# arpitbansal297/Cold-Diffusion-Models

Hardware: AMD Instinct MI355X
Metric: unet_train_imgs_per_sec (higher is better)
Workload: dtype f32 storage/accumulate; dense-conv GEMM operands bf16x3; 1 GPU; CelebA-128 denoising cold diffusion (BASELINE config 3): Unet(dim=64,(1,2,4,8),ch=3) @128x128, T=200, optimizer step = 2 micro-batches x 32 img (one fused forward / backward pass over all of them: same draws, same gradient sum) + Adam + EMA/10; per_gpu_batch=32, gradient_accumulate_every=2, parallelism=single

## Files before the change

cold-diffusion-models_amd/csrc/k_pack.hip:

```cpp
#include "cdf_common.h"
#include "colddiff.h"

__global__ void pack_weight_kernel(const float* src, float* dst, int T, int R, int C, int ldc, long long s_t,
                                   long long s_r, long long s_c) {
    const long long n = (long long)T * R * ldc;
    for (long long i = (long long)blockIdx.x * blockDim.x + threadIdx.x; i < n; i += (long long)gridDim.x * blockDim.x) {
        const int c = (int)(i % ldc);
        const long long tr = i / ldc;
        const int r = (int)(tr % R), t = (int)(tr / R);
        dst[i] = c < C ? src[c * s_c + r * s_r + t * s_t] : 0.f;
    }
}

__global__ void pack_weight_bf16_kernel(const float* src, unsigned short* dst_hi, unsigned short* dst_lo, int T, int R, int C,
                                        int ldc, long long s_t, long long s_r, long long s_c) {
    const long long n = (long long)T * R * ldc;
    for (long long i = (long long)blockIdx.x * blockDim.x + threadIdx.x; i < n; i += (long long)gridDim.x * blockDim.x) {
        const int c = (int)(i % ldc);
        const long long tr = i / ldc;
        const int r = (int)(tr % R), t = (int)(tr / R);
        const float v = c < C ? src[c * s_c + r * s_r + t * s_t] : 0.f;
        const unsigned h = cdf_f2bf(v);
        dst_hi[i] = (unsigned short)h;
        if (dst_lo) dst_lo[i] = (unsigned short)cdf_f2bf(v - cdf_bf2f(h));
    }
}

__global__ void split_bf16_kernel(const float* x, int ldx, unsigned short* hi, unsigned short* lo, int ldo, long long rows, int C4) {
    const long long n = rows * C4;
    for (long long i = (long long)blockIdx.x * blockDim.x + threadIdx.x; i < n; i += (long long)gridDim.x * blockDim.x) {
        const int c = (int)(i % C4) * 4;
        const long long r = i / C4;
        const float4 v = *(const float4*)(x + r * ldx + c);
        uint2 h, l;
        cdf_split4(v.x, v.y, v.z, v.w, h, l);
        *(uint2*)(hi + r * ldo + c) = h;
        if (lo) *(uint2*)(lo + r * ldo + c) = l;
    }
}

__global__ void widen_bf16_kernel(const unsigned short* x, int ldx, float* y, int ldy, long long rows, int C4) {
    const long long n = rows * C4;
    for (long long i = (long long)blockIdx.x * blockDim.x + threadIdx.x; i < n; i += (long long)gridDim.x * blockDim.x) {
        const int c = (int)(i % C4) * 4;
        const long long r = i / C4;
        *(float4*)(y + r * ldy + c) = cdf_quad_cvt(*(const uint2*)(x + r * ldx + c));
    }
}

struct CdfPackEntry {
    const float* src;
    void* dst0;
    void* dst1;
    long long s_t, s_r, s_c;
    int T, R, C, ldc, kind, first_block;
};

__global__ void __launch_bounds__(256) pack_many_kernel(const CdfPackEntry* tab, int nentries) {
    int lo = 0, hi = nentries - 1;
    const int b = blockIdx.x;
    while (lo < hi) {
        const int mid = (lo + hi + 1) >> 1;
        if (tab[mid].first_block <= b) lo = mid; else hi = mid - 1;
    }
    const CdfPackEntry e = tab[lo];
    if (e.s_t == 1 && e.T > 1 && e.T <= 16) {
        const long long n2 = (long long)e.R * e.ldc;
        const long long j0 = (long long)(b - e.first_block) * 1024 + threadIdx.x;
        const long long plane = (long long)e.R * e.ldc;
#pragma unroll
        for (int k = 0; k < 4; ++k) {
            const long long j = j0 + 256 * k;
            if (j >= n2) break;
            const int c = (int)(j % e.ldc), r = (int)(j / e.ldc);
            const bool ok = c < e.C;
            const float* sp = e.src + (ok ? c * e.s_c + r * e.s_r : 0);
            float v[16];
#pragma unroll
            for (int t = 0; t < 16; ++t) v[t] = sp[t < e.T ? t : 0];
#pragma unroll
            for (int t = 0; t < 16; ++t) {
                if (t >= e.T) break;
                const float x = ok ? v[t] : 0.f;
                const long long i = t * plane + j;
                if (e.kind == 0) {
                    ((float*)e.dst0)[i] = x;
                } else {
                    const unsigned h = cdf_f2bf(x);
                    ((unsigned short*)e.dst0)[i] = (unsigned short)h;
                    if (e.dst1) ((unsigned short*)e.dst1)[i] = (unsigned short)cdf_f2bf(x - cdf_bf2f(h));
                }
            }
        }
        return;
    }
    const long long n = (long long)e.T * e.R * e.ldc;
    const long long i0 = (long long)(b - e.first_block) * 1024 + threadIdx.x;
#pragma unroll
    for (int k = 0; k < 4; ++k) {
        const long long i = i0 + 256 * k;
        if (i >= n) break;
        const int c = (int)(i % e.ldc);
        const long long tr = i / e.ldc;
        const int r = (int)(tr % e.R), t = (int)(tr / e.R);
        const float v = c < e.C ? e.src[c * e.s_c + r * e.s_r + t * e.s_t] : 0.f;
        if (e.kind == 0) {
            ((float*)e.dst0)[i] = v;
        } else {
            const unsigned h = cdf_f2bf(v);
            ((unsigned short*)e.dst0)[i] = (unsigned short)h;
            if (e.dst1) ((unsigned short*)e.dst1)[i] = (unsigned short)cdf_f2bf(v - cdf_bf2f(h));
        }
    }
}

extern "C" int cdf_pack_entry_bytes(void) { return (int)sizeof(CdfPackEntry); }
extern "C" int cdf_pack_blocks(int T, int R, int ldc, long long s_t) {
    const long long n = (s_t == 1 && T > 1 && T <= 16) ? (long long)R * ldc : (long long)T * R * ldc;
    return (int)((n + 1023) / 1024);
}

extern "C" int cdf_pack_many(const void* table, int nentries, int nblocks, void* stream) {
    CDF_REQUIRE(table && nentries > 0 && nblocks > 0, "cdf_pack_many: bad args");
    CDF_LAUNCH(pack_many_kernel, dim3(nblocks), dim3(256), 0, CDF_S, (const CdfPackEntry*)table, nentries);
    return cdf_check_launch("pack_many");
}

extern "C" int cdf_pack_weight(const float* src, float* dst, int T, int R, int C, int ldc, long long s_t,
                               long long s_r, long long s_c, void* stream) {
    CDF_REQUIRE(src && dst && T > 0 && R > 0 && C > 0 && ldc >= C && ldc % 4 == 0, "cdf_pack_weight: bad args");
    CDF_LAUNCH(pack_weight_kernel, dim3(cdf_ew_grid4k((long long)T * R * ldc)), dim3(256), 0, CDF_S, src, dst, T, R, C, ldc, s_t, s_r, s_c);
    return cdf_check_launch("pack_weight");
}

extern "C" int cdf_pack_weight_bf16(const float* src, void* dst_hi, void* dst_lo, int T, int R, int C, int ldc, long long s_t,
                                    long long s_r, long long s_c, void* stream) {
    CDF_REQUIRE(src && dst_hi && T > 0 && R > 0 && C > 0 && ldc >= C && ldc % 32 == 0, "cdf_pack_weight_bf16: bad args (ldc must be a multiple of 32)");
    long long g = ((long long)T * R * ldc + 255) / 256;
    if (g > 4096) g = 4096;
    CDF_LAUNCH(pack_weight_bf16_kernel, dim3((int)g), dim3(256), 0, CDF_S, src, (unsigned short*)dst_hi, (unsigned short*)dst_lo, T, R, C, ldc, s_t, s_r, s_c);
    return cdf_check_launch("pack_weight_bf16");
}

extern "C" int cdf_split_bf16(const float* x, int ldx, void* hi, void* lo, int ldo, long long rows, int C, void* stream) {
    CDF_REQUIRE(x && hi && rows > 0 && C > 0 && C % 4 == 0 && ldx % 4 == 0 && ldo % 8 == 0 && ldo >= C, "cdf_split_bf16: bad args (C %% 4, ldo %% 8)");
    long long g = (rows * (C / 4) + 255) / 256;
    if (g > 8192) g = 8192;
    CDF_LAUNCH(split_bf16_kernel, dim3((int)g), dim3(256), 0, CDF_S, x, ldx, (unsigned short*)hi, (unsigned short*)lo, ldo, rows, C / 4);
    return cdf_check_launch("split_bf16");
}

extern "C" int cdf_bf16_to_f32(const void* x, int ldx, float* y, int ldy, long long rows, int C, void* stream) {
    CDF_REQUIRE(x && y && rows > 0 && C > 0 && C % 4 == 0 && ldx % 4 == 0 && ldy % 4 == 0 && ldx >= C && ldy >= C && (((uintptr_t)x) & 7) == 0 &&
                (((uintptr_t)y) & 15) == 0, "cdf_bf16_to_f32: bad args (C %% 4, pitches %% 4, x 8-byte / y 16-byte aligned)");
    long long g = (rows * (C / 4) + 255) / 256;
    if (g > 8192) g = 8192;
    CDF_LAUNCH(widen_bf16_kernel, dim3((int)g), dim3(256), 0, CDF_S, (const unsigned short*)x, ldx, y, ldy, rows, C / 4);
    return cdf_check_launch("bf16_to_f32");
}
```

Before: 1334 img/s.

## Tile weight packing through shared memory for coalesced reads and vector writes

Replaces the per-element strided gather in the batched weight-pack kernel with a 3D tiled transpose staged in shared memory. The loop dimensions are sorted by source stride so global reads stay as contiguous as possible, and the output is written as float4 or packed uint4 bf16 hi/lo vectors. The aim is to cut uncoalesced memory traffic when converting weights into GEMM layouts each step. It adds shared-memory use, more index arithmetic and a different block-count formula that the host side must stay consistent with.

```diff
diff --git a/cold-diffusion-models_amd/csrc/k_pack.hip b/cold-diffusion-models_amd/csrc/k_pack.hip
--- a/cold-diffusion-models_amd/csrc/k_pack.hip
+++ b/cold-diffusion-models_amd/csrc/k_pack.hip
@@ -56,7 +56,17 @@
     int T, R, C, ldc, kind, first_block;
 };
 
+#define PACK_TC 32
+#define PACK_ROWS 288
+#define PACK_LP (PACK_TC + 1)
+static __host__ __device__ inline void pack_tile(int T, int& RE, int& TE) {
+    TE = T < 64 ? T : 64;
+    RE = PACK_ROWS / TE;
+    if (RE > 128) RE = 128;
+}
+
 __global__ void __launch_bounds__(256) pack_many_kernel(const CdfPackEntry* tab, int nentries) {
+    __shared__ float tile[PACK_ROWS * PACK_LP];
     int lo = 0, hi = nentries - 1;
     const int b = blockIdx.x;
     while (lo < hi) {
@@ -64,60 +74,124 @@
         if (tab[mid].first_block <= b) lo = mid; else hi = mid - 1;
     }
     const CdfPackEntry e = tab[lo];
-    if (e.s_t == 1 && e.T > 1 && e.T <= 16) {
-        const long long n2 = (long long)e.R * e.ldc;
-        const long long j0 = (long long)(b - e.first_block) * 1024 + threadIdx.x;
-        const long long plane = (long long)e.R * e.ldc;
-#pragma unroll
-        for (int k = 0; k < 4; ++k) {
-            const long long j = j0 + 256 * k;
-            if (j >= n2) break;
-            const int c = (int)(j % e.ldc), r = (int)(j / e.ldc);
-            const bool ok = c < e.C;
-            const float* sp = e.src + (ok ? c * e.s_c + r * e.s_r : 0);
-            float v[16];
-#pragma unroll
-            for (int t = 0; t < 16; ++t) v[t] = sp[t < e.T ? t : 0];
-#pragma unroll
-            for (int t = 0; t < 16; ++t) {
-                if (t >= e.T) break;
-                const float x = ok ? v[t] : 0.f;
-                const long long i = t * plane + j;
-                if (e.kind == 0) {
-                    ((float*)e.dst0)[i] = x;
-                } else {
-                    const unsigned h = cdf_f2bf(x);
-                    ((unsigned short*)e.dst0)[i] = (unsigned short)h;
-                    if (e.dst1) ((unsigned short*)e.dst1)[i] = (unsigned short)cdf_f2bf(x - cdf_bf2f(h));
+    int RE, TE;
+    pack_tile(e.T, RE, TE);
+    const int tiles_c = (e.ldc + PACK_TC - 1) / PACK_TC, tiles_r = (e.R + RE - 1) / RE;
+    int bid = b - e.first_block;
+    const int c0 = (bid % tiles_c) * PACK_TC;
+    bid /= tiles_c;
+    const int r0 = (bid % tiles_r) * RE, t0 = (bid / tiles_r) * TE;
+    const int tid = threadIdx.x;
+
+    {
+        int e0 = PACK_TC, e1 = RE, e2 = TE;
+        int s0 = (int)e.s_c, s1 = (int)e.s_r, s2 = (int)e.s_t;
+        int l0 = 1, l1 = PACK_LP, l2 = RE * PACK_LP;
+        int m0 = e.C - c0, m1 = e.R - r0, m2 = e.T - t0;
+        auto key = [](int s, int ext) { return ext == 1 ? 0x7fffffff : s; };
+        auto cswap = [&](int& ea, int& sa, int& la, int& ma, int& eb, int& sb, int& lb, int& mb) {
+            if (key(sb, eb) < key(sa, ea)) {
+                int t_;
+                t_ = ea; ea = eb; eb = t_;
+                t_ = sa; sa = sb; sb = t_;
+                t_ = la; la = lb; lb = t_;
+                t_ = ma; ma = mb; mb = t_;
+            }
+        };
+        cswap(e0, s0, l0, m0, e1, s1, l1, m1);
+        cswap(e1, s1, l1, m1, e2, s2, l2, m2);
+        cswap(e0, s0, l0, m0, e1, s1, l1, m1);
+        const int n = PACK_TC * RE * TE;
+        int a0 = tid % e0, a1 = (tid / e0) % e1, a2 = tid / (e0 * e1);
+        const int d0 = 256 % e0, d1 = (256 / e0) % e1, d2 = 256 / (e0 * e1);
+        const float* sp = e.C > c0 ? e.src + ((long long)c0 * e.s_c + (long long)r0 * e.s_r + (long long)t0 * e.s_t) : e.src;
+        const int D = d0 * s0 + d1 * s1 + d2 * s2, W0 = s1 - e0 * s0, W1 = s2 - e1 * s1;
+        const int DL = d0 * l0 + d1 * l1 + d2 * l2, WL0 = l1 - e0 * l0, WL1 = l2 - e1 * l1;
+        constexpr int NI = PACK_TC * PACK_ROWS / 256;
+        float v[NI];
+        {
+            int b0 = a0, b1 = a1, b2 = a2;
+            int off = a0 * s0 + a1 * s1 + a2 * s2;
+#pragma unroll
+            for (int k = 0; k < NI; ++k) {
+                const bool ok = tid + 256 * k < n && b0 < m0 && b1 < m1 && b2 < m2;
+                const float x = sp[ok ? off : 0];
+                v[k] = ok ? x : 0.f;
+                b0 += d0; b1 += d1; b2 += d2;
+                off += D;
+                if (b0 >= e0) { b0 -= e0; ++b1; off += W0; }
+                if (b1 >= e1) { b1 -= e1; ++b2; off += W1; }
+            }
+        }
+        int lof = a0 * l0 + a1 * l1 + a2 * l2;
+#pragma unroll
+        for (int k = 0; k < NI; ++k) {
+            if (tid + 256 * k < n) tile[lof] = v[k];
+            a0 += d0; a1 += d1;
+            lof += DL;
+            if (a0 >= e0) { a0 -= e0; ++a1; lof += WL0; }
+            if (a1 >= e1) { a1 -= e1; lof += WL1; }
+        }
+    }
+    __syncthreads();
+
+    const int rows = RE * TE;
+    const int rlim = e.R - r0, tlim = e.T - t0;
+    if (e.kind == 0) {
+        float* dst = (float*)e.dst0;
+        const bool vec = ((((uintptr_t)dst) & 15) == 0) && (e.ldc & 3) == 0;
+        for (int v = tid; v < rows * (PACK_TC / 4); v += 256) {
+            const int row = v >> 3, cl = (v & 7) * 4;
+            const int tl = row / RE, rl = row - tl * RE, c = c0 + cl;
+            if (tl >= tlim || rl >= rlim || c >= e.ldc) continue;
+            const float* tp = tile + row * PACK_LP + cl;
+            float* dp = dst + ((long long)(t0 + tl) * e.R + (r0 + rl)) * e.ldc + c;
+            if (vec) {
+                *(float4*)dp = make_float4(tp[0], tp[1], tp[2], tp[3]);
+            } else {
+#pragma unroll
+                for (int k = 0; k < 4; ++k)
+                    if (c + k < e.ldc) dp[k] = tp[k];
+            }
+        }
+    } else {
+        unsigned short* dhi = (unsigned short*)e.dst0;
+        unsigned short* dlo = (unsigned short*)e.dst1;
+        const bool vec = (((((uintptr_t)dhi) | ((uintptr_t)dlo)) & 15) == 0) && (e.ldc & 7) == 0;
+        for (int v = tid; v < rows * (PACK_TC / 8); v += 256) {
+            const int row = v >> 2, cl = (v & 3) * 8;
+            const int tl = row / RE, rl = row - tl * RE, c = c0 + cl;
+            if (tl >= tlim || rl >= rlim || c >= e.ldc) continue;
+            const float* tp = tile + row * PACK_LP + cl;
+            const long long di = ((long long)(t0 + tl) * e.R + (r0 + rl)) * e.ldc + c;
+            unsigned h[8], l[8];
+#pragma unroll
+            for (int k = 0; k < 8; ++k) {
+                const float x = tp[k];
+                h[k] = cdf_f2bf(x);
+                l[k] = cdf_f2bf(x - cdf_bf2f(h[k]));
+            }
+            if (vec) {
+                *(uint4*)(dhi + di) = make_uint4(h[0] | (h[1] << 16), h[2] | (h[3] << 16), h[4] | (h[5] << 16), h[6] | (h[7] << 16));
+                if (dlo) *(uint4*)(dlo + di) = make_uint4(l[0] | (l[1] << 16), l[2] | (l[3] << 16), l[4] | (l[5] << 16), l[6] | (l[7] << 16));
+            } else {
+#pragma unroll
+                for (int k = 0; k < 8; ++k) {
+                    if (c + k >= e.ldc) break;
+                    dhi[di + k] = (unsigned short)h[k];
+                    if (dlo) dlo[di + k] = (unsigned short)l[k];
                 }
             }
-        }
-        return;
-    }
-    const long long n = (long long)e.T * e.R * e.ldc;
-    const long long i0 = (long long)(b - e.first_block) * 1024 + threadIdx.x;
-#pragma unroll
-    for (int k = 0; k < 4; ++k) {
-        const long long i = i0 + 256 * k;
-        if (i >= n) break;
-        const int c = (int)(i % e.ldc);
-        const long long tr = i / e.ldc;
-        const int r = (int)(tr % e.R), t = (int)(tr / e.R);
-        const float v = c < e.C ? e.src[c * e.s_c + r * e.s_r + t * e.s_t] : 0.f;
-        if (e.kind == 0) {
-            ((float*)e.dst0)[i] = v;
-        } else {
-            const unsigned h = cdf_f2bf(v);
-            ((unsigned short*)e.dst0)[i] = (unsigned short)h;
-            if (e.dst1) ((unsigned short*)e.dst1)[i] = (unsigned short)cdf_f2bf(v - cdf_bf2f(h));
         }
     }
 }
 
 extern "C" int cdf_pack_entry_bytes(void) { return (int)sizeof(CdfPackEntry); }
 extern "C" int cdf_pack_blocks(int T, int R, int ldc, long long s_t) {
-    const long long n = (s_t == 1 && T > 1 && T <= 16) ? (long long)R * ldc : (long long)T * R * ldc;
-    return (int)((n + 1023) / 1024);
+    (void)s_t;
+    int RE, TE;
+    pack_tile(T, RE, TE);
+    return (int)((long long)((ldc + PACK_TC - 1) / PACK_TC) * ((R + RE - 1) / RE) * ((T + TE - 1) / TE));
 }
 
 extern "C" int cdf_pack_many(const void* table, int nentries, int nblocks, void* stream) {
```

Result: no change. 1337 img/s (median of 6 runs) (+0.2%).
